# nagadomi/nunif

Hardware: NVIDIA H100
Metric: waifu2x_input_megapixels_per_sec (higher is better)
Workload: dtype f16

## Files before the change

### nunif_b200/csrc/gemm.cu

```cuda
#include "gemm.h"
#include "gemm_wgmma.cuh"
#include "tmap.h"
#include "../../include/nunif_b200.h"
#include <mutex>
#include <cstdlib>

namespace nb200 {

typedef CUresult (*EncodeTiledFn)(CUtensorMap*, CUtensorMapDataType, cuuint32_t, void*, const cuuint64_t*,
                                  const cuuint64_t*, const cuuint32_t*, const cuuint32_t*, CUtensorMapInterleave,
                                  CUtensorMapSwizzle, CUtensorMapL2promotion, CUtensorMapFloatOOBfill);

static EncodeTiledFn get_encode() {
    static EncodeTiledFn fn = nullptr;
    static std::once_flag once;
    std::call_once(once, [] {
        void* p = nullptr;
        cudaDriverEntryPointQueryResult q;
        if (cudaGetDriverEntryPoint("cuTensorMapEncodeTiled", &p, cudaEnableDefault, &q) == cudaSuccess &&
            q == cudaDriverEntryPointSuccess)
            fn = (EncodeTiledFn)p;
    });
    return fn;
}

int encode(CUtensorMap* m, const void* base, int rank, const cuuint64_t* dims, const cuuint64_t* strides_bytes,
                  const cuuint32_t* box, int swizzle_bytes) {
    EncodeTiledFn fn = get_encode();
    if (!fn) return fail("cuTensorMapEncodeTiled is not available (no CUDA driver?)");
    cuuint32_t estr[5] = {1, 1, 1, 1, 1};
    CUtensorMapSwizzle sw = swizzle_bytes == 128 ? CU_TENSOR_MAP_SWIZZLE_128B
                                                 : (swizzle_bytes == 64 ? CU_TENSOR_MAP_SWIZZLE_64B : CU_TENSOR_MAP_SWIZZLE_32B);
    CUresult r = fn(m, CU_TENSOR_MAP_DATA_TYPE_FLOAT16, (cuuint32_t)rank, const_cast<void*>(base), dims, strides_bytes, box,
                    estr, CU_TENSOR_MAP_INTERLEAVE_NONE, sw, CU_TENSOR_MAP_L2_PROMOTION_L2_256B,
                    CU_TENSOR_MAP_FLOAT_OOB_FILL_NONE);
    if (r != CUDA_SUCCESS) return fail("cuTensorMapEncodeTiled failed with CUresult " + std::to_string((int)r));
    return 0;
}

template <int BN, int BK, bool A2 = false>
static int launch_t(cudaStream_t st, const GemmMaps& maps, const GemmParams& p, int m_tiles, int n_tiles) {
    using Cfg = GemmCfg<BN, BK>;
    if (ensure_dyn_smem((const void*)gemm_conv_kernel<BN, BK, A2>, Cfg::SMEM_BYTES)) return 1;
    cudaLaunchConfig_t cfg = {};
    cfg.gridDim = dim3((unsigned)m_tiles * n_tiles); cfg.blockDim = dim3(GEMM_THREADS); cfg.dynamicSmemBytes = Cfg::SMEM_BYTES;
    cfg.stream = st;
    cudaLaunchAttribute at[1];
    at[0].id = cudaLaunchAttributeProgrammaticStreamSerialization;
    at[0].val.programmaticStreamSerializationAllowed = 1;
    cfg.attrs = at; cfg.numAttrs = 1;
    NB_CUDA(cudaLaunchKernelEx(&cfg, gemm_conv_kernel<BN, BK, A2>, maps, p));
    NB_LAUNCHED();
    return 0;
}

template <int BK>
static int launch_bn(int bn, cudaStream_t st, const GemmMaps& maps, const GemmParams& p, int m_tiles, int n_tiles) {
    if (p.k2) switch (bn) {
        case 64: return launch_t<64, BK, true>(st, maps, p, m_tiles, n_tiles);
        case 96: return launch_t<96, BK, true>(st, maps, p, m_tiles, n_tiles);
        default: return fail("second A operand: unsupported BLOCK_N");
    }
    switch (bn) {
        case 16: return launch_t<16, BK>(st, maps, p, m_tiles, n_tiles);
        case 32: return launch_t<32, BK>(st, maps, p, m_tiles, n_tiles);
        case 48: return launch_t<48, BK>(st, maps, p, m_tiles, n_tiles);
        case 64: return launch_t<64, BK>(st, maps, p, m_tiles, n_tiles);
        case 96: return launch_t<96, BK>(st, maps, p, m_tiles, n_tiles);
        case 128: return launch_t<128, BK>(st, maps, p, m_tiles, n_tiles);
    }
    return fail("unsupported BLOCK_N");
}

static int num_sms() { return device_sm_count(); }

std::atomic<int> g_tune_epoch{0};
int g_tune[16] = {0, 0, 0,  0, 0, 0,  0,
                   0, 0,  0,
                   0,
                   0, 0, 0, 0, 0};

static int encode_nhwc4(CUtensorMap* m, const __half* base, int C, int X, int Y, int B, long long sx, long long sy, long long sb,
                        int cw, int tw, int th) {
    cuuint64_t dims[4] = {(cuuint64_t)C, (cuuint64_t)X, (cuuint64_t)Y, (cuuint64_t)B};
    cuuint64_t strides[3] = {(cuuint64_t)sx * 2, (cuuint64_t)sy * 2, (cuuint64_t)sb * 2};
    cuuint32_t box[4] = {(cuuint32_t)cw, (cuuint32_t)tw, (cuuint32_t)th, 1};
    return encode(m, base, 4, dims, strides, box, cw * 2);
}

int conv_gemm(cudaStream_t st, const ConvGemm& g) {
    NB_CHECK(g.A && g.Wt && g.out, "null pointer");
    NB_CHECK(g.Ci % 8 == 0, "input channel stride must be a multiple of 8");
    NB_CHECK(g.N % 16 == 0, "N must be a multiple of 16 (pad the weights)");
    GemmParams p;
    memset(&p, 0, sizeof(p));
    int ktap;
    cuuint64_t dims[5], strides[4];
    cuuint32_t box[5];
    const cuuint64_t e = 2;
    const cuuint64_t rs = (g.a_row_stride ? (cuuint64_t)g.a_row_stride : (cuuint64_t)g.Wi * g.Ci) * e;
    const cuuint64_t is = (g.a_img_stride ? (cuuint64_t)g.a_img_stride * e : (cuuint64_t)g.Hi * rs);
    switch (g.kind) {
        case CG_LINEAR_FLAT: {
            const long long M = (long long)g.B * g.Hi * g.Wi;
            p.B = 1; p.Ho = 1; p.Wo = (int)M; p.TH = 1; p.TW = 128;
            p.taps = g.a_planes; ktap = g.Cin;
            NB_CHECK(g.a_planes >= 1 && g.a_planes <= 16, "bad plane count");
            for (int t = 0; t < p.taps; ++t) { p.tap_dy[t] = 0; p.tap_dx[t] = 0; p.tap_dyi[t] = (int8_t)t; }
            dims[0] = g.Cin; dims[1] = M; dims[2] = g.a_planes; dims[3] = 1; dims[4] = 1;
            strides[0] = g.Ci * e; strides[1] = (g.a_planes > 1 ? (cuuint64_t)g.a_plane_stride : (cuuint64_t)M * g.Ci) * e;
            strides[2] = (cuuint64_t)M * g.Ci * e * g.a_planes; strides[3] = strides[2];
            break;
        }
        case CG_LINEAR_2D:
        case CG_CONV3: {
            const int kk = g.kind == CG_CONV3 ? 3 : 1;
            const int pad = g.kind == CG_CONV3 ? g.pad : 0;
            NB_CHECK(pad == 0 || pad == 1, "conv3x3 padding must be 0 or 1");
            p.B = g.B; p.Ho = g.Hi - (kk - 1) + 2 * pad; p.Wo = g.Wi - (kk - 1) + 2 * pad; p.TH = 8; p.TW = 16;
            p.taps = kk * kk; ktap = g.Cin;
            for (int t = 0; t < p.taps; ++t) { p.tap_dy[t] = (int8_t)(t / kk - pad); p.tap_dx[t] = (int8_t)(t % kk - pad); p.tap_dyi[t] = 0; }
            dims[0] = g.Cin; dims[1] = g.Wi; dims[2] = 1; dims[3] = g.Hi; dims[4] = g.B;
            strides[0] = g.Ci * e; strides[1] = rs; strides[2] = rs;
            strides[3] = is;
            break;
        }
        case CG_TCONV3: {
            NB_CHECK(g.dil >= 1 && g.dil <= 127, "temporal dilation must be in [1, 127]");
            p.B = g.B; p.Ho = g.Hi; p.Wo = g.Wi; p.TH = 8; p.TW = 16;
            p.taps = 3; ktap = g.Cin;
            for (int t = 0; t < 3; ++t) { p.tap_dy[t] = (int8_t)((t - 1) * g.dil); p.tap_dx[t] = 0; p.tap_dyi[t] = 0; }
            dims[0] = g.Cin; dims[1] = g.Wi; dims[2] = 1; dims[3] = g.Hi; dims[4] = g.B;
            strides[0] = g.Ci * e; strides[1] = rs; strides[2] = rs;
// ... 56 lines not shown
            if (c >= bn || g.N % c) continue;
            const int w = (c % 64 == 0) ? 64 : 32;
            if (split && g.cout % w) continue;
            bn = c; cw = w;
        }
    }
    p.n_tiles = g.N / bn;
    box[0] = BK; box[1] = p.TW; box[2] = 1; box[3] = p.TH; box[4] = 1;
    GemmMaps maps;
    memset(&maps, 0, sizeof(maps));
    if (encode(&maps.a, g.A, 5, dims, strides, box, BK * 2)) return 1;
    const int K = p.taps * ktap + (a2 ? g.Cin2 : 0);
    cuuint64_t bdims[2] = {(cuuint64_t)K, (cuuint64_t)g.N};
    cuuint64_t bstr[1] = {(cuuint64_t)K * e};
    cuuint32_t bbox[2] = {(cuuint32_t)BK, (cuuint32_t)bn};
    if (encode(&maps.b, g.Wt, 2, bdims, bstr, bbox, BK * 2)) return 1;
    if (split) {
        for (int q = 0; q < g.N / g.cout; ++q)
            if (encode_nhwc4(&maps.o[q], g.out + (size_t)q * g.split_stride, g.cout, p.Wo, p.Ho, p.B, g.ldo, (long long)p.Wo * g.ldo,
                             (long long)p.Ho * p.Wo * g.ldo, cw, p.TW, p.TH)) return 1;
    } else if (!shuf) {
        if (encode_nhwc4(&maps.o[0], g.out, g.N, p.Wo, p.Ho, p.B, g.ldo, (long long)p.Wo * g.ldo, (long long)p.Ho * p.Wo * g.ldo,
                         cw, p.TW, p.TH)) return 1;
        if (g.res) {
            const int rW = g.kind == CG_LINEAR_FLAT ? p.Wo : g.res_W, rH = g.kind == CG_LINEAR_FLAT ? 1 : g.res_H;
            p.res_cx = g.kind == CG_LINEAR_FLAT ? 0 : g.res_cx;
            p.res_cy = g.kind == CG_LINEAR_FLAT ? 0 : g.res_cy;
            if (encode_nhwc4(&maps.r[0], g.res, g.N, rW, rH, p.B, g.ldr, (long long)rW * g.ldr, (long long)rH * rW * g.ldr, cw,
                             p.TW, p.TH)) return 1;
        }
    } else {
        const int OW = 2 * p.Wo, OH = 2 * p.Ho;
        for (int q = 0; q < 4; ++q) {
            const int dy = q >> 1, dx = q & 1;
            if (encode_nhwc4(&maps.o[q], g.out + ((size_t)dy * OW + dx) * g.ldo, g.cout, p.Wo, p.Ho, p.B, 2LL * g.ldo,
                             2LL * OW * g.ldo, (long long)OH * OW * g.ldo, cw, p.TW, p.TH)) return 1;
            if (g.res) {
                const int oy = dy + g.res_cy, ox = dx + g.res_cx;
                NB_CHECK(oy + 2 * (p.Ho - 1) < g.res_H && ox + 2 * (p.Wo - 1) < g.res_W, "residual tensor too small");
                if (encode_nhwc4(&maps.r[q], g.res + ((size_t)oy * g.res_W + ox) * g.ldr, g.cout, p.Wo, p.Ho, p.B, 2LL * g.ldr,
                                 2LL * g.res_W * g.ldr, (long long)g.res_H * g.res_W * g.ldr, cw, p.TW, p.TH)) return 1;
            }
        }
        p.res_cx = p.res_cy = 0;
        if (a2) {
            const cuuint64_t px = (cuuint64_t)g.ld2 * e;
            cuuint64_t d2[5] = {(cuuint64_t)g.Cin2, 2, (cuuint64_t)p.Wo, 2, (cuuint64_t)p.B * p.Ho};
            cuuint64_t s2[4] = {px, 2 * px, (cuuint64_t)OW * px, 2 * (cuuint64_t)OW * px};
            cuuint32_t b2[5] = {(cuuint32_t)BK, 1, (cuuint32_t)p.TW, 1, (cuuint32_t)p.TH};
            if (encode(&maps.a2, g.A2, 5, d2, s2, b2, BK * 2)) return 1;
        }
    }
    const int m_tiles = p.tiles_x * p.tiles_y * p.B;
    const double Mrows = (double)p.B * p.Ho * p.Wo;
    const double in_px = g.kind == CG_DOWN2 ? 4.0 * Mrows : ((g.kind == CG_CONV3 || g.kind == CG_TCONV3) ? (double)p.B * g.Hi * g.Wi : Mrows);
    ProfScope ps(st, PC_GEMM, 2.0 * Mrows * (double)g.N * (double)K,
                 in_px * (g.kind == CG_LINEAR_FLAT ? g.Cin * g.a_planes : g.Cin) * 2.0 + (g.res ? Mrows * g.N * 2.0 : 0.0) +
                     4.0 * Mrows * g.Cin2 * (a2 ? 2.0 : 0.0) + (double)g.N * K * 2.0,
                 Mrows * (double)g.N * 2.0);
    if (rec_on())
        rec_launch("gemm", {{"kind", g.kind}, {"pad", g.pad}, {"dil", g.dil}, {"B", g.B}, {"Hi", g.Hi}, {"Wi", g.Wi}, {"Ci", g.Ci},
                            {"Cin", g.Cin}, {"a_row_stride", g.a_row_stride}, {"a_img_stride", g.a_img_stride},
                            {"a_planes", g.a_planes}, {"a_plane_stride", g.a_plane_stride}, {"N", g.N}, {"act", g.act},
                            {"ldo", g.ldo}, {"out_mode", g.out_mode}, {"cout", g.cout}, {"split_stride", g.split_stride},
                            {"has_bias", g.bias ? 1 : 0}, {"has_res", g.res ? 1 : 0}, {"ldr", g.ldr}, {"res_H", g.res_H},
                            {"res_W", g.res_W}, {"res_cy", g.res_cy}, {"res_cx", g.res_cx}, {"res_before_act", g.res_before_act},
                            {"has_a2", a2 ? 1 : 0}, {"Cin2", g.Cin2}, {"ld2", g.ld2},
                            {"out_is_res", g.res && (const void*)g.out == (const void*)g.res},
                            {"out_is_a", (const void*)g.out == (const void*)g.A}, {"block_n", bn}, {"bk", BK},
                            {"grid", m_tiles * p.n_tiles}});
    return BK == 64 ? launch_bn<64>(bn, st, maps, p, m_tiles, p.n_tiles) : launch_bn<32>(bn, st, maps, p, m_tiles, p.n_tiles);
}

}

using namespace nb200;

extern "C" int nb200_conv_gemm_f16(const void* A, int B, int Hi, int Wi, int Ci, int Cin, int kind, const void* Wt, int N,
                                   const float* bias, int act, void* out, int ldo, int out_mode, int cout,
                                   const void* res, int ldr, int res_H, int res_W, int res_cy, int res_cx,
                                   int res_before_act, void* stream) {
    ConvGemm g;
    g.A = (const __half*)A; g.B = B; g.Hi = Hi; g.Wi = Wi; g.Ci = Ci; g.Cin = Cin;
    g.kind = kind == 4 ? CG_CONV3 : kind;
    g.pad = kind == 4 ? 1 : 0;
    g.Wt = (const __half*)Wt; g.N = N; g.bias = bias; g.act = act; g.out = (__half*)out; g.ldo = ldo;
    g.out_mode = out_mode; g.cout = cout; g.res = (const __half*)res; g.ldr = ldr; g.res_H = res_H; g.res_W = res_W;
    g.res_cy = res_cy; g.res_cx = res_cx; g.res_before_act = res_before_act;
    return conv_gemm((cudaStream_t)stream, g);
}

extern "C" int nb200_conv_gemm_pixshuf_a2_f16(const void* A, int B, int Hi, int Wi, int Ci, const void* Wt, int N, const float* bias,
                                              int act, void* out, int ldo, int cout, const void* A2, int Cin2, int ld2, void* stream) {
    ConvGemm g;
    g.A = (const __half*)A; g.B = B; g.Hi = Hi; g.Wi = Wi; g.Ci = Ci; g.Cin = Ci; g.kind = CG_LINEAR_2D;
    g.Wt = (const __half*)Wt; g.N = N; g.bias = bias; g.act = act; g.out = (__half*)out; g.ldo = ldo;
    g.out_mode = OUT_PIXSHUF2; g.cout = cout; g.A2 = (const __half*)A2; g.Cin2 = Cin2; g.ld2 = ld2;
    NB_CHECK(g.A2, "null pointer");
    return conv_gemm((cudaStream_t)stream, g);
}

extern "C" int nb200_conv_gemm_ex_f16(const nb200_gemm_desc* d, const void* A, const void* Wt, const float* bias, void* out,
                                      const void* res, const void* A2, void* stream) {
    NB_CHECK(d, "null descriptor");
    ConvGemm g;
    g.A = (const __half*)A; g.B = d->B; g.Hi = d->Hi; g.Wi = d->Wi; g.Ci = d->Ci; g.Cin = d->Cin;
    g.a_row_stride = d->a_row_stride; g.a_img_stride = d->a_img_stride; g.kind = d->kind; g.pad = d->pad; g.dil = d->dil;
    g.Wt = (const __half*)Wt; g.N = d->N; g.bias = bias; g.act = d->act; g.out = (__half*)out; g.ldo = d->ldo;
    g.out_mode = d->out_mode; g.cout = d->cout; g.split_stride = d->split_stride; g.a_planes = d->a_planes;
    g.a_plane_stride = d->a_plane_stride; g.res = (const __half*)res; g.ldr = d->ldr; g.res_H = d->res_H; g.res_W = d->res_W;
    g.res_cy = d->res_cy; g.res_cx = d->res_cx; g.res_before_act = d->res_before_act;
    g.A2 = (const __half*)A2; g.Cin2 = d->Cin2; g.ld2 = d->ld2;
    return conv_gemm((cudaStream_t)stream, g);
}

extern "C" int nb200_tune_set(int key, int value) {
    NB_CHECK(key >= 0 && key < 16, "bad key");
    g_tune[key] = value;
    g_tune_epoch.fetch_add(1);
    return 0;
}
```

### nunif_b200/csrc/gemm_wgmma.cuh

```cuda
#pragma once
#include "common.cuh"
#include "ptx.cuh"
#include <cuda.h>

namespace nb200 {

enum : int { ACT_NONE = 0, ACT_LRELU01 = 1, ACT_GELU = 2, ACT_RELU = 3 };
enum : int { OUT_NHWC = 0, OUT_PIXSHUF2 = 1, OUT_SPLIT = 2 };

struct GemmParams {
    int B, Ho, Wo, TH, TW, tiles_x, tiles_y;
    int N;
    int taps, cpt;
    int8_t tap_dx[16], tap_dy[16], tap_dyi[16];
    int n_tiles;
    const float* bias;
    int act;
    int out_mode, cout;
    int has_res, res_cy, res_cx;
    int res_before_act;
    int k2;
};

struct GemmMaps {
// ... 121 lines not shown
template <> __device__ __forceinline__ void wgmma_f16<128>(float (&d)[64], uint64_t a, uint64_t b, uint32_t acc) {
    asm volatile("{\n\t.reg .pred p;\n\tsetp.ne.b32 p, %66, 0;\n\t"
                 "wgmma.mma_async.sync.aligned.m64n128k16.f32.f16.f16 {%0, %1, %2, %3, %4, %5, %6, %7, %8, %9, %10, %11, %12, %13, %14, %15, %16, %17, %18, %19, %20, %21, %22, %23, %24, %25, %26, %27, %28, %29, %30, %31, %32, %33, %34, %35, %36, %37, %38, %39, %40, %41, %42, %43, %44, %45, %46, %47, %48, %49, %50, %51, %52, %53, %54, %55, %56, %57, %58, %59, %60, %61, %62, %63}, %64, %65, p, 1, 1, 0, 0;\n\t}"
                 : "+f"(d[0]), "+f"(d[1]), "+f"(d[2]), "+f"(d[3]), "+f"(d[4]), "+f"(d[5]), "+f"(d[6]), "+f"(d[7]), "+f"(d[8]), "+f"(d[9]), "+f"(d[10]), "+f"(d[11]), "+f"(d[12]), "+f"(d[13]), "+f"(d[14]), "+f"(d[15]), "+f"(d[16]), "+f"(d[17]), "+f"(d[18]), "+f"(d[19]), "+f"(d[20]), "+f"(d[21]), "+f"(d[22]), "+f"(d[23]), "+f"(d[24]), "+f"(d[25]), "+f"(d[26]), "+f"(d[27]), "+f"(d[28]), "+f"(d[29]), "+f"(d[30]), "+f"(d[31]), "+f"(d[32]), "+f"(d[33]), "+f"(d[34]), "+f"(d[35]), "+f"(d[36]), "+f"(d[37]), "+f"(d[38]), "+f"(d[39]), "+f"(d[40]), "+f"(d[41]), "+f"(d[42]), "+f"(d[43]), "+f"(d[44]), "+f"(d[45]), "+f"(d[46]), "+f"(d[47]), "+f"(d[48]), "+f"(d[49]), "+f"(d[50]), "+f"(d[51]), "+f"(d[52]), "+f"(d[53]), "+f"(d[54]), "+f"(d[55]), "+f"(d[56]), "+f"(d[57]), "+f"(d[58]), "+f"(d[59]), "+f"(d[60]), "+f"(d[61]), "+f"(d[62]), "+f"(d[63])
                 : "l"(a), "l"(b), "r"(acc));
}

__device__ __forceinline__ void wgmma_f16_rs96(float (&d)[48], const uint32_t (&a)[4], uint64_t b, uint32_t acc) {
    asm volatile("{\n\t.reg .pred p;\n\tsetp.ne.b32 p, %53, 0;\n\t"
                 "wgmma.mma_async.sync.aligned.m64n96k16.f32.f16.f16 {%0, %1, %2, %3, %4, %5, %6, %7, %8, %9, %10, %11, %12, %13, %14, %15, %16, %17, %18, %19, %20, %21, %22, %23, %24, %25, %26, %27, %28, %29, %30, %31, %32, %33, %34, %35, %36, %37, %38, %39, %40, %41, %42, %43, %44, %45, %46, %47}, {%48, %49, %50, %51}, %52, p, 1, 1, 0;\n\t}"
                 : "+f"(d[0]), "+f"(d[1]), "+f"(d[2]), "+f"(d[3]), "+f"(d[4]), "+f"(d[5]), "+f"(d[6]), "+f"(d[7]), "+f"(d[8]), "+f"(d[9]), "+f"(d[10]), "+f"(d[11]), "+f"(d[12]), "+f"(d[13]), "+f"(d[14]), "+f"(d[15]), "+f"(d[16]), "+f"(d[17]), "+f"(d[18]), "+f"(d[19]), "+f"(d[20]), "+f"(d[21]), "+f"(d[22]), "+f"(d[23]), "+f"(d[24]), "+f"(d[25]), "+f"(d[26]), "+f"(d[27]), "+f"(d[28]), "+f"(d[29]), "+f"(d[30]), "+f"(d[31]), "+f"(d[32]), "+f"(d[33]), "+f"(d[34]), "+f"(d[35]), "+f"(d[36]), "+f"(d[37]), "+f"(d[38]), "+f"(d[39]), "+f"(d[40]), "+f"(d[41]), "+f"(d[42]), "+f"(d[43]), "+f"(d[44]), "+f"(d[45]), "+f"(d[46]), "+f"(d[47])
                 : "r"(a[0]), "r"(a[1]), "r"(a[2]), "r"(a[3]), "l"(b), "r"(acc));
}

__device__ __forceinline__ float gelu_erf(float x) {
    const float a = fabsf(x);
    float q = fmaf(a, 4.88118734e-04f, -7.19881030e-03f);
    q = fmaf(q, a, 5.21468017e-02f);
    q = fmaf(q, a, 4.59595724e-01f);
    q = fmaf(q, a, 1.15100057e+00f);
    const float e = ex2(fmaf(-q, a, -1.0f));
    return fmaxf(x, 0.f) - a * e;
}

template <int K>
__device__ __forceinline__ void apply_act(float (&v)[K], int act) {
    switch (act) {
        case ACT_LRELU01:
#pragma unroll
            for (int j = 0; j < K; ++j) v[j] = v[j] > 0.f ? v[j] : 0.1f * v[j];
            break;
        case ACT_GELU:
#pragma unroll
            for (int j = 0; j < K; ++j) v[j] = gelu_erf(v[j]);
            break;
        case ACT_RELU:
#pragma unroll
            for (int j = 0; j < K; ++j) v[j] = fmaxf(v[j], 0.f);
            break;
        default: break;
    }
}

constexpr int GEMM_CONSUMER_THREADS = 256;
constexpr int GEMM_THREADS = GEMM_CONSUMER_THREADS + 32;

template <int BLOCK_N, int BK>
struct GemmCfg {
    static_assert(BLOCK_N % 16 == 0 && BLOCK_N <= 128, "BLOCK_N: 16..128 (the fp32 accumulators live in registers)");
    static constexpr int SWIZZLE = BK * 2;
    static constexpr int A_BYTES = 128 * BK * 2;
    static constexpr int B_BYTES = BLOCK_N * BK * 2;
    static constexpr int STAGE_BYTES = A_BYTES + ((B_BYTES + 1023) / 1024) * 1024;
    static constexpr int STAGES = (98304 / STAGE_BYTES) < 2 ? 2 : ((98304 / STAGE_BYTES) > 6 ? 6 : (98304 / STAGE_BYTES));
    static constexpr int CW = (BLOCK_N % 64 == 0) ? 64 : ((BLOCK_N % 32 == 0) ? 32 : 16);
    static constexpr int NCH = BLOCK_N / CW;
    static constexpr int CH_BYTES = 128 * CW * 2;
    static_assert(NCH * CH_BYTES <= STAGES * STAGE_BYTES, "epilogue staging must fit in the (drained) pipeline stages");
    static constexpr int SMEM_BYTES = STAGES * STAGE_BYTES + 1024  + 256 ;
};

template <int CW>
__device__ __forceinline__ uint32_t stage_off(int r, int j) {
    if (CW == 64) return (uint32_t)(r * 128 + ((j ^ (r & 7)) << 4));
    if (CW == 32) return (uint32_t)(r * 64 + ((j ^ ((r >> 1) & 3)) << 4));
    return (uint32_t)(r * 32 + ((j ^ ((r >> 2) & 1)) << 4));
}

template <int ROWS>
__device__ __forceinline__ uint32_t sw64_off(int r, int col) {
    return (uint32_t)((col >> 5) * (ROWS * 64)) + stage_off<32>(r, (col & 31) >> 3) + (uint32_t)((col & 7) * 2);
}

template <int BLOCK_N, int BK, bool A2 = false>
__global__ void __launch_bounds__(GEMM_THREADS, 2) gemm_conv_kernel(const __grid_constant__ GemmMaps maps,
                                                                    const __grid_constant__ GemmParams p) {
    using Cfg = GemmCfg<BLOCK_N, BK>;
    constexpr int STAGES = Cfg::STAGES;
    constexpr int CW = Cfg::CW;
    extern __shared__ uint8_t smem_dyn[];
    uint8_t* smem = reinterpret_cast<uint8_t*>((reinterpret_cast<uintptr_t>(smem_dyn) + 1023) & ~(uintptr_t)1023);
    uint64_t* full_bar = reinterpret_cast<uint64_t*>(smem + STAGES * Cfg::STAGE_BYTES);
    uint64_t* empty_bar = full_bar + STAGES;
    uint64_t* res_bar = empty_bar + STAGES;

    const int warp = threadIdx.x >> 5;
    const int n_tile = blockIdx.x % p.n_tiles;
    const int tile = blockIdx.x / p.n_tiles;
    const int tx_i = tile % p.tiles_x;
    const int ty_i = (tile / p.tiles_x) % p.tiles_y;
    const int b = tile / (p.tiles_x * p.tiles_y);
    const int x0 = tx_i * p.TW, y0 = ty_i * p.TH;
    const int n0 = n_tile * BLOCK_N;
    const int k_iters = p.taps * p.cpt + (A2 ? p.k2 : 0);

    if (threadIdx.x == GEMM_CONSUMER_THREADS) {
        tma_prefetch_desc(&maps.a);
        tma_prefetch_desc(&maps.b);
        tma_prefetch_desc(&maps.o[0]);
        for (int s = 0; s < STAGES; ++s) {
            mbar_init(&full_bar[s], 1);
            mbar_init(&empty_bar[s], 2);
        }
        mbar_init(res_bar, 1);
        fence_barrier_init();
    }
    __syncthreads();

    if (warp == GEMM_CONSUMER_THREADS / 32) {
        if (elect_one()) {
            asm volatile("griddepcontrol.wait;" ::: "memory");
            for (int it = 0; it < k_iters; ++it) {
                const int s = it % STAGES;
                const uint32_t ph = (it / STAGES) & 1;
                mbar_wait(&empty_bar[s], ph ^ 1);
                const int tap = it / p.cpt, ch = it - tap * p.cpt;
                uint8_t* sa = smem + s * Cfg::STAGE_BYTES;
                uint8_t* sb = sa + Cfg::A_BYTES;
                mbar_expect_tx(&full_bar[s], Cfg::A_BYTES + Cfg::B_BYTES);
                if (A2 && tap >= p.taps) {
                    const int q = n0 / p.cout;
                    tma_load_5d(&maps.a2, &full_bar[s], sa, (it - p.taps * p.cpt) * BK, q & 1, x0, q >> 1, b * p.Ho + y0);
                } else {
                    tma_load_5d(&maps.a, &full_bar[s], sa, ch * BK, x0 + p.tap_dx[tap], p.tap_dyi[tap], y0 + p.tap_dy[tap], b);
                }
                tma_load_2d(&maps.b, &full_bar[s], sb, it * BK, n0);
            }
        }
        return;
    }

    const int wg = threadIdx.x >> 7;
    const int t = threadIdx.x & 127;
    float acc[BLOCK_N / 2];
#pragma unroll
    for (int j = 0; j < BLOCK_N / 2; ++j) acc[j] = 0.f;
    for (int it = 0; it < k_iters; ++it) {
        const int s = it % STAGES;
        mbar_wait(&full_bar[s], (it / STAGES) & 1);
        const uint32_t sa = smem_u32(smem + s * Cfg::STAGE_BYTES) + wg * 64 * Cfg::SWIZZLE;
        const uint32_t sb = smem_u32(smem + s * Cfg::STAGE_BYTES) + Cfg::A_BYTES;
        wgmma_fence();
#pragma unroll
        for (int k = 0; k < BK / 16; ++k)
            wgmma_f16<BLOCK_N>(acc, make_kmajor_desc<Cfg::SWIZZLE>(sa + k * 32), make_kmajor_desc<Cfg::SWIZZLE>(sb + k * 32), 1u);
        wgmma_commit();
        wgmma_wait<1>();
        if (it > 0 && t == 0) mbar_arrive(&empty_bar[(it - 1) % STAGES]);
    }
    wgmma_wait<0>();
    wgmma_fence_operands(acc);
    if (threadIdx.x == 0) NB_PDL_TRIGGER();
    consumer_bar_sync();
    uint8_t* stg = smem;
    const bool leader = threadIdx.x == 0;
    if (p.has_res) {
        if (leader) {
            mbar_expect_tx(res_bar, Cfg::NCH * Cfg::CH_BYTES);
#pragma unroll 1
            for (int c = 0; c < Cfg::NCH; ++c) {
                const int n = n0 + c * CW;
                const int g = p.out_mode != OUT_NHWC ? n / p.cout : 0;
                const int co = p.out_mode != OUT_NHWC ? n - g * p.cout : n;
                tma_load_4d(&maps.r[g], res_bar, stg + c * Cfg::CH_BYTES, co, x0 + p.res_cx, y0 + p.res_cy, b);
            }
        }
        mbar_wait(res_bar, 0);
    }
    const int act = p.act;
    const bool has_res = p.has_res != 0, res_first = p.res_before_act != 0;
    const int row0 = wg * 64 + (t >> 5) * 16 + ((t & 31) >> 2);
    const int cq = 2 * (t & 3);
#pragma unroll
    for (int j = 0; j < BLOCK_N / 8; ++j) {
        const int col = 8 * j + cq;
        const int c = (8 * j) / CW;
        float2 bq = make_float2(0.f, 0.f);
        if (p.bias) bq = __ldg(reinterpret_cast<const float2*>(p.bias + n0 + col));
        float v[4] = {acc[4 * j] + bq.x, acc[4 * j + 1] + bq.y, acc[4 * j + 2] + bq.x, acc[4 * j + 3] + bq.y};
        __half2* s0 = reinterpret_cast<__half2*>(stg + c * Cfg::CH_BYTES + stage_off<CW>(row0, (8 * j % CW) / 8) + 2 * cq);
        __half2* s1 = reinterpret_cast<__half2*>(stg + c * Cfg::CH_BYTES + stage_off<CW>(row0 + 8, (8 * j % CW) / 8) + 2 * cq);
        if (has_res) {
            const float2 r0 = __half22float2(*s0), r1 = __half22float2(*s1);
            const float rv[4] = {r0.x, r0.y, r1.x, r1.y};
            if (res_first) {
#pragma unroll
                for (int q = 0; q < 4; ++q) v[q] += rv[q];
                apply_act(v, act);
            } else {
                apply_act(v, act);
#pragma unroll
                for (int q = 0; q < 4; ++q) v[q] += rv[q];
            }
        } else {
            apply_act(v, act);
        }
        *s0 = __floats2half2_rn(v[0], v[1]);
        *s1 = __floats2half2_rn(v[2], v[3]);
    }
    fence_async_smem();
    consumer_bar_sync();
    if (leader) {
#pragma unroll 1
        for (int c = 0; c < Cfg::NCH; ++c) {
            const int n = n0 + c * CW;
            const int g = p.out_mode != OUT_NHWC ? n / p.cout : 0;
            const int co = p.out_mode != OUT_NHWC ? n - g * p.cout : n;
            tma_store_4d(&maps.o[g], stg + c * Cfg::CH_BYTES, co, x0, y0, b);
        }
        tma_store_commit();
        tma_store_wait_read();
    }
}

}
```

Baseline: 79.55.

## Make wgmma conv GEMM persistent with dedicated epilogue staging buffer

Turns the conv GEMM kernel into a persistent kernel. The grid is capped at two CTAs per SM and each CTA loops over tiles, so the producer's TMA ring keeps prefetching the next tile while the consumers run the epilogue. A separate staging buffer for the epilogue lets output TMA stores overlap with the next tile's mainloop, and the PDL trigger moves to kernel start. The trade-off is fewer pipeline stages, since shared memory is sized for two CTAs per SM, plus extra cross-tile barrier phase tracking that could hurt small or low-tile-count layers.

```diff
diff --git a/nunif_b200/csrc/gemm.cu b/nunif_b200/csrc/gemm.cu
--- a/nunif_b200/csrc/gemm.cu
+++ b/nunif_b200/csrc/gemm.cu
@@ -2,6 +2,7 @@
 #include "gemm_wgmma.cuh"
 #include "tmap.h"
 #include "../../include/nunif_b200.h"
+#include <algorithm>
 #include <mutex>
 #include <cstdlib>
 
@@ -39,11 +40,11 @@
 }
 
 template <int BN, int BK, bool A2 = false>
-static int launch_t(cudaStream_t st, const GemmMaps& maps, const GemmParams& p, int m_tiles, int n_tiles) {
+static int launch_t(cudaStream_t st, const GemmMaps& maps, const GemmParams& p, int grid) {
     using Cfg = GemmCfg<BN, BK>;
     if (ensure_dyn_smem((const void*)gemm_conv_kernel<BN, BK, A2>, Cfg::SMEM_BYTES)) return 1;
     cudaLaunchConfig_t cfg = {};
-    cfg.gridDim = dim3((unsigned)m_tiles * n_tiles); cfg.blockDim = dim3(GEMM_THREADS); cfg.dynamicSmemBytes = Cfg::SMEM_BYTES;
+    cfg.gridDim = dim3((unsigned)grid); cfg.blockDim = dim3(GEMM_THREADS); cfg.dynamicSmemBytes = Cfg::SMEM_BYTES;
     cfg.stream = st;
     cudaLaunchAttribute at[1];
     at[0].id = cudaLaunchAttributeProgrammaticStreamSerialization;
@@ -55,19 +56,19 @@
 }
 
 template <int BK>
-static int launch_bn(int bn, cudaStream_t st, const GemmMaps& maps, const GemmParams& p, int m_tiles, int n_tiles) {
+static int launch_bn(int bn, cudaStream_t st, const GemmMaps& maps, const GemmParams& p, int grid) {
     if (p.k2) switch (bn) {
-        case 64: return launch_t<64, BK, true>(st, maps, p, m_tiles, n_tiles);
-        case 96: return launch_t<96, BK, true>(st, maps, p, m_tiles, n_tiles);
+        case 64: return launch_t<64, BK, true>(st, maps, p, grid);
+        case 96: return launch_t<96, BK, true>(st, maps, p, grid);
         default: return fail("second A operand: unsupported BLOCK_N");
     }
     switch (bn) {
-        case 16: return launch_t<16, BK>(st, maps, p, m_tiles, n_tiles);
-        case 32: return launch_t<32, BK>(st, maps, p, m_tiles, n_tiles);
-        case 48: return launch_t<48, BK>(st, maps, p, m_tiles, n_tiles);
-        case 64: return launch_t<64, BK>(st, maps, p, m_tiles, n_tiles);
-        case 96: return launch_t<96, BK>(st, maps, p, m_tiles, n_tiles);
-        case 128: return launch_t<128, BK>(st, maps, p, m_tiles, n_tiles);
+        case 16: return launch_t<16, BK>(st, maps, p, grid);
+        case 32: return launch_t<32, BK>(st, maps, p, grid);
+        case 48: return launch_t<48, BK>(st, maps, p, grid);
+        case 64: return launch_t<64, BK>(st, maps, p, grid);
+        case 96: return launch_t<96, BK>(st, maps, p, grid);
+        case 128: return launch_t<128, BK>(st, maps, p, grid);
     }
     return fail("unsupported BLOCK_N");
 }
@@ -78,7 +79,8 @@
 int g_tune[16] = {0, 0, 0,  0, 0, 0,  0,
                    0, 0,  0,
                    0,
-                   0, 0, 0, 0, 0};
+                   0,
+                   0, 0, 0, 0};
 
 static int encode_nhwc4(CUtensorMap* m, const __half* base, int C, int X, int Y, int B, long long sx, long long sy, long long sb,
                         int cw, int tw, int th) {
@@ -241,6 +243,8 @@
         }
     }
     const int m_tiles = p.tiles_x * p.tiles_y * p.B;
+    int grid = std::min(m_tiles * p.n_tiles, 2 * num_sms());
+    if (g_tune[12] > 0) grid = std::min(grid, g_tune[12]);
     const double Mrows = (double)p.B * p.Ho * p.Wo;
     const double in_px = g.kind == CG_DOWN2 ? 4.0 * Mrows : ((g.kind == CG_CONV3 || g.kind == CG_TCONV3) ? (double)p.B * g.Hi * g.Wi : Mrows);
     ProfScope ps(st, PC_GEMM, 2.0 * Mrows * (double)g.N * (double)K,
@@ -257,8 +261,8 @@
                             {"has_a2", a2 ? 1 : 0}, {"Cin2", g.Cin2}, {"ld2", g.ld2},
                             {"out_is_res", g.res && (const void*)g.out == (const void*)g.res},
                             {"out_is_a", (const void*)g.out == (const void*)g.A}, {"block_n", bn}, {"bk", BK},
-                            {"grid", m_tiles * p.n_tiles}});
-    return BK == 64 ? launch_bn<64>(bn, st, maps, p, m_tiles, p.n_tiles) : launch_bn<32>(bn, st, maps, p, m_tiles, p.n_tiles);
+                            {"grid", grid}});
+    return BK == 64 ? launch_bn<64>(bn, st, maps, p, grid) : launch_bn<32>(bn, st, maps, p, grid);
 }
 
 }
diff --git a/nunif_b200/csrc/gemm_wgmma.cuh b/nunif_b200/csrc/gemm_wgmma.cuh
--- a/nunif_b200/csrc/gemm_wgmma.cuh
+++ b/nunif_b200/csrc/gemm_wgmma.cuh
@@ -197,12 +197,16 @@
     static constexpr int A_BYTES = 128 * BK * 2;
     static constexpr int B_BYTES = BLOCK_N * BK * 2;
     static constexpr int STAGE_BYTES = A_BYTES + ((B_BYTES + 1023) / 1024) * 1024;
-    static constexpr int STAGES = (98304 / STAGE_BYTES) < 2 ? 2 : ((98304 / STAGE_BYTES) > 6 ? 6 : (98304 / STAGE_BYTES));
     static constexpr int CW = (BLOCK_N % 64 == 0) ? 64 : ((BLOCK_N % 32 == 0) ? 32 : 16);
     static constexpr int NCH = BLOCK_N / CW;
     static constexpr int CH_BYTES = 128 * CW * 2;
-    static_assert(NCH * CH_BYTES <= STAGES * STAGE_BYTES, "epilogue staging must fit in the (drained) pipeline stages");
-    static constexpr int SMEM_BYTES = STAGES * STAGE_BYTES + 1024  + 256 ;
+    static constexpr int STG_BYTES = NCH * CH_BYTES;
+    static constexpr int SMEM_PER_CTA = (228 * 1024 - 2 * 1024) / 2;
+    static constexpr int RING_FIT = (SMEM_PER_CTA - 1024  - 256  - STG_BYTES) / STAGE_BYTES;
+    static constexpr int STAGES = RING_FIT > 6 ? 6 : RING_FIT;
+    static_assert(STAGES >= 2, "the ring needs two stages beside the staging tile");
+    static constexpr int SMEM_BYTES = STAGES * STAGE_BYTES + STG_BYTES + 1024  + 256 ;
+    static_assert(SMEM_BYTES <= SMEM_PER_CTA, "two CTAs per SM");
 };
 
 template <int CW>
@@ -215,6 +219,16 @@
 template <int ROWS>
 __device__ __forceinline__ uint32_t sw64_off(int r, int col) {
     return (uint32_t)((col >> 5) * (ROWS * 64)) + stage_off<32>(r, (col & 31) >> 3) + (uint32_t)((col & 7) * 2);
+}
+
+struct GemmTile { int x0, y0, b, n0; };
+template <int BLOCK_N>
+__device__ __forceinline__ GemmTile gemm_tile(const GemmParams& p, int idx) {
+    const int n_tile = idx % p.n_tiles;
+    const int tile = idx / p.n_tiles;
+    const int tx_i = tile % p.tiles_x;
+    const int ty_i = (tile / p.tiles_x) % p.tiles_y;
+    return {tx_i * p.TW, ty_i * p.TH, tile / (p.tiles_x * p.tiles_y), n_tile * BLOCK_N};
 }
 
 template <int BLOCK_N, int BK, bool A2 = false>
@@ -225,18 +239,13 @@
     constexpr int CW = Cfg::CW;
     extern __shared__ uint8_t smem_dyn[];
     uint8_t* smem = reinterpret_cast<uint8_t*>((reinterpret_cast<uintptr_t>(smem_dyn) + 1023) & ~(uintptr_t)1023);
-    uint64_t* full_bar = reinterpret_cast<uint64_t*>(smem + STAGES * Cfg::STAGE_BYTES);
+    uint8_t* stg = smem + STAGES * Cfg::STAGE_BYTES;
+    uint64_t* full_bar = reinterpret_cast<uint64_t*>(stg + Cfg::STG_BYTES);
     uint64_t* empty_bar = full_bar + STAGES;
     uint64_t* res_bar = empty_bar + STAGES;
 
     const int warp = threadIdx.x >> 5;
-    const int n_tile = blockIdx.x % p.n_tiles;
-    const int tile = blockIdx.x / p.n_tiles;
-    const int tx_i = tile % p.tiles_x;
-    const int ty_i = (tile / p.tiles_x) % p.tiles_y;
-    const int b = tile / (p.tiles_x * p.tiles_y);
-    const int x0 = tx_i * p.TW, y0 = ty_i * p.TH;
-    const int n0 = n_tile * BLOCK_N;
+    const int n_tiles_all = p.tiles_x * p.tiles_y * p.B * p.n_tiles;
     const int k_iters = p.taps * p.cpt + (A2 ? p.k2 : 0);
 
     if (threadIdx.x == GEMM_CONSUMER_THREADS) {
@@ -251,25 +260,34 @@
         fence_barrier_init();
     }
     __syncthreads();
+    if (threadIdx.x == 0) NB_PDL_TRIGGER();
 
     if (warp == GEMM_CONSUMER_THREADS / 32) {
         if (elect_one()) {
             asm volatile("griddepcontrol.wait;" ::: "memory");
-            for (int it = 0; it < k_iters; ++it) {
-                const int s = it % STAGES;
-                const uint32_t ph = (it / STAGES) & 1;
-                mbar_wait(&empty_bar[s], ph ^ 1);
-                const int tap = it / p.cpt, ch = it - tap * p.cpt;
-                uint8_t* sa = smem + s * Cfg::STAGE_BYTES;
-                uint8_t* sb = sa + Cfg::A_BYTES;
-                mbar_expect_tx(&full_bar[s], Cfg::A_BYTES + Cfg::B_BYTES);
-                if (A2 && tap >= p.taps) {
-                    const int q = n0 / p.cout;
-                    tma_load_5d(&maps.a2, &full_bar[s], sa, (it - p.taps * p.cpt) * BK, q & 1, x0, q >> 1, b * p.Ho + y0);
-                } else {
-                    tma_load_5d(&maps.a, &full_bar[s], sa, ch * BK, x0 + p.tap_dx[tap], p.tap_dyi[tap], y0 + p.tap_dy[tap], b);
+            int s = 0;
+            uint32_t ph = 0;
+#pragma unroll 1
+            for (int idx = blockIdx.x; idx < n_tiles_all; idx += gridDim.x) {
+                const GemmTile tl = gemm_tile<BLOCK_N>(p, idx);
+#pragma unroll 1
+                for (int it = 0; it < k_iters; ++it) {
+                    mbar_wait(&empty_bar[s], ph ^ 1);
+                    const int tap = it / p.cpt, ch = it - tap * p.cpt;
+                    uint8_t* sa = smem + s * Cfg::STAGE_BYTES;
+                    uint8_t* sb = sa + Cfg::A_BYTES;
+                    mbar_expect_tx(&full_bar[s], Cfg::A_BYTES + Cfg::B_BYTES);
+                    if (A2 && tap >= p.taps) {
+                        const int q = tl.n0 / p.cout;
+                        tma_load_5d(&maps.a2, &full_bar[s], sa, (it - p.taps * p.cpt) * BK, q & 1, tl.x0, q >> 1,
+                                    tl.b * p.Ho + tl.y0);
+                    } else {
+                        tma_load_5d(&maps.a, &full_bar[s], sa, ch * BK, tl.x0 + p.tap_dx[tap], p.tap_dyi[tap],
+                                    tl.y0 + p.tap_dy[tap], tl.b);
+                    }
+                    tma_load_2d(&maps.b, &full_bar[s], sb, it * BK, tl.n0);
+                    if (++s == STAGES) { s = 0; ph ^= 1; }
                 }
-                tma_load_2d(&maps.b, &full_bar[s], sb, it * BK, n0);
             }
         }
         return;
@@ -277,85 +295,95 @@
 
     const int wg = threadIdx.x >> 7;
     const int t = threadIdx.x & 127;
-    float acc[BLOCK_N / 2];
-#pragma unroll
-    for (int j = 0; j < BLOCK_N / 2; ++j) acc[j] = 0.f;
-    for (int it = 0; it < k_iters; ++it) {
-        const int s = it % STAGES;
-        mbar_wait(&full_bar[s], (it / STAGES) & 1);
-        const uint32_t sa = smem_u32(smem + s * Cfg::STAGE_BYTES) + wg * 64 * Cfg::SWIZZLE;
-        const uint32_t sb = smem_u32(smem + s * Cfg::STAGE_BYTES) + Cfg::A_BYTES;
-        wgmma_fence();
-#pragma unroll
-        for (int k = 0; k < BK / 16; ++k)
-            wgmma_f16<BLOCK_N>(acc, make_kmajor_desc<Cfg::SWIZZLE>(sa + k * 32), make_kmajor_desc<Cfg::SWIZZLE>(sb + k * 32), 1u);
-        wgmma_commit();
-        wgmma_wait<1>();
-        if (it > 0 && t == 0) mbar_arrive(&empty_bar[(it - 1) % STAGES]);
-    }
-    wgmma_wait<0>();
-    wgmma_fence_operands(acc);
-    if (threadIdx.x == 0) NB_PDL_TRIGGER();
-    consumer_bar_sync();
-    uint8_t* stg = smem;
     const bool leader = threadIdx.x == 0;
-    if (p.has_res) {
-        if (leader) {
-            mbar_expect_tx(res_bar, Cfg::NCH * Cfg::CH_BYTES);
-#pragma unroll 1
-            for (int c = 0; c < Cfg::NCH; ++c) {
-                const int n = n0 + c * CW;
-                const int g = p.out_mode != OUT_NHWC ? n / p.cout : 0;
-                const int co = p.out_mode != OUT_NHWC ? n - g * p.cout : n;
-                tma_load_4d(&maps.r[g], res_bar, stg + c * Cfg::CH_BYTES, co, x0 + p.res_cx, y0 + p.res_cy, b);
-            }
-        }
-        mbar_wait(res_bar, 0);
-    }
     const int act = p.act;
     const bool has_res = p.has_res != 0, res_first = p.res_before_act != 0;
     const int row0 = wg * 64 + (t >> 5) * 16 + ((t & 31) >> 2);
     const int cq = 2 * (t & 3);
-#pragma unroll
-    for (int j = 0; j < BLOCK_N / 8; ++j) {
-        const int col = 8 * j + cq;
-        const int c = (8 * j) / CW;
-        float2 bq = make_float2(0.f, 0.f);
-        if (p.bias) bq = __ldg(reinterpret_cast<const float2*>(p.bias + n0 + col));
-        float v[4] = {acc[4 * j] + bq.x, acc[4 * j + 1] + bq.y, acc[4 * j + 2] + bq.x, acc[4 * j + 3] + bq.y};
-        __half2* s0 = reinterpret_cast<__half2*>(stg + c * Cfg::CH_BYTES + stage_off<CW>(row0, (8 * j % CW) / 8) + 2 * cq);
-        __half2* s1 = reinterpret_cast<__half2*>(stg + c * Cfg::CH_BYTES + stage_off<CW>(row0 + 8, (8 * j % CW) / 8) + 2 * cq);
+    int s = 0;
+    uint32_t ph = 0, res_ph = 0;
+#pragma unroll 1
+    for (int idx = blockIdx.x; idx < n_tiles_all; idx += gridDim.x) {
+        const GemmTile tl = gemm_tile<BLOCK_N>(p, idx);
+        float acc[BLOCK_N / 2];
+#pragma unroll
+        for (int j = 0; j < BLOCK_N / 2; ++j) acc[j] = 0.f;
+        int prev = 0;
+        for (int it = 0; it < k_iters; ++it) {
+            mbar_wait(&full_bar[s], ph);
+            const uint32_t sa = smem_u32(smem + s * Cfg::STAGE_BYTES) + wg * 64 * Cfg::SWIZZLE;
+            const uint32_t sb = smem_u32(smem + s * Cfg::STAGE_BYTES) + Cfg::A_BYTES;
+            wgmma_fence();
+#pragma unroll
+            for (int k = 0; k < BK / 16; ++k)
+                wgmma_f16<BLOCK_N>(acc, make_kmajor_desc<Cfg::SWIZZLE>(sa + k * 32), make_kmajor_desc<Cfg::SWIZZLE>(sb + k * 32), 1u);
+            wgmma_commit();
+            wgmma_wait<1>();
+            if (it > 0 && t == 0) mbar_arrive(&empty_bar[prev]);
+            prev = s;
+            if (++s == STAGES) { s = 0; ph ^= 1; }
+        }
+        wgmma_wait<0>();
+        wgmma_fence_operands(acc);
+        if (t == 0) mbar_arrive(&empty_bar[prev]);
+
+        if (leader) tma_store_wait_read();
+        consumer_bar_sync();
         if (has_res) {
-            const float2 r0 = __half22float2(*s0), r1 = __half22float2(*s1);
-            const float rv[4] = {r0.x, r0.y, r1.x, r1.y};
-            if (res_first) {
-#pragma unroll
-                for (int q = 0; q < 4; ++q) v[q] += rv[q];
-                apply_act(v, act);
+            if (leader) {
+                mbar_expect_tx(res_bar, Cfg::STG_BYTES);
+#pragma unroll 1
+                for (int c = 0; c < Cfg::NCH; ++c) {
+                    const int n = tl.n0 + c * CW;
+                    const int g = p.out_mode != OUT_NHWC ? n / p.cout : 0;
+                    const int co = p.out_mode != OUT_NHWC ? n - g * p.cout : n;
+                    tma_load_4d(&maps.r[g], res_bar, stg + c * Cfg::CH_BYTES, co, tl.x0 + p.res_cx, tl.y0 + p.res_cy, tl.b);
+                }
+            }
+            mbar_wait(res_bar, res_ph);
+            res_ph ^= 1;
+        }
+#pragma unroll
+        for (int j = 0; j < BLOCK_N / 8; ++j) {
+            const int col = 8 * j + cq;
+            const int c = (8 * j) / CW;
+            float2 bq = make_float2(0.f, 0.f);
+            if (p.bias) bq = __ldg(reinterpret_cast<const float2*>(p.bias + tl.n0 + col));
+            float v[4] = {acc[4 * j] + bq.x, acc[4 * j + 1] + bq.y, acc[4 * j + 2] + bq.x, acc[4 * j + 3] + bq.y};
+            __half2* s0 = reinterpret_cast<__half2*>(stg + c * Cfg::CH_BYTES + stage_off<CW>(row0, (8 * j % CW) / 8) + 2 * cq);
+            __half2* s1 = reinterpret_cast<__half2*>(stg + c * Cfg::CH_BYTES + stage_off<CW>(row0 + 8, (8 * j % CW) / 8) + 2 * cq);
+            if (has_res) {
+                const float2 r0 = __half22float2(*s0), r1 = __half22float2(*s1);
+                const float rv[4] = {r0.x, r0.y, r1.x, r1.y};
+                if (res_first) {
+#pragma unroll
+                    for (int q = 0; q < 4; ++q) v[q] += rv[q];
+                    apply_act(v, act);
+                } else {
+                    apply_act(v, act);
+#pragma unroll
+                    for (int q = 0; q < 4; ++q) v[q] += rv[q];
+                }
             } else {
                 apply_act(v, act);
-#pragma unroll
-                for (int q = 0; q < 4; ++q) v[q] += rv[q];
             }
-        } else {
-            apply_act(v, act);
-        }
-        *s0 = __floats2half2_rn(v[0], v[1]);
-        *s1 = __floats2half2_rn(v[2], v[3]);
+            *s0 = __floats2half2_rn(v[0], v[1]);
+            *s1 = __floats2half2_rn(v[2], v[3]);
+        }
+        fence_async_smem();
+        consumer_bar_sync();
+        if (leader) {
+#pragma unroll 1
+            for (int c = 0; c < Cfg::NCH; ++c) {
+                const int n = tl.n0 + c * CW;
+                const int g = p.out_mode != OUT_NHWC ? n / p.cout : 0;
+                const int co = p.out_mode != OUT_NHWC ? n - g * p.cout : n;
+                tma_store_4d(&maps.o[g], stg + c * Cfg::CH_BYTES, co, tl.x0, tl.y0, tl.b);
+            }
+            tma_store_commit();
+        }
     }
-    fence_async_smem();
-    consumer_bar_sync();
-    if (leader) {
-#pragma unroll 1
-        for (int c = 0; c < Cfg::NCH; ++c) {
-            const int n = n0 + c * CW;
-            const int g = p.out_mode != OUT_NHWC ? n / p.cout : 0;
-            const int co = p.out_mode != OUT_NHWC ? n - g * p.cout : n;
-            tma_store_4d(&maps.o[g], stg + c * Cfg::CH_BYTES, co, x0, y0, b);
-        }
-        tma_store_commit();
-        tma_store_wait_read();
-    }
-}
-
-}
+    if (leader) tma_store_wait_read();
+}
+
+}
diff --git a/profiles/ab_gemm.py b/profiles/ab_gemm.py
--- /dev/null
+++ b/profiles/ab_gemm.py
@@ -0,0 +1,185 @@
+#!/usr/bin/env python
+import argparse
+import ctypes
+import json
+import os
+import statistics
+import subprocess
+import sys
+
+ROOT = os.path.dirname(os.path.dirname(os.path.abspath(__file__)))
+sys.path.insert(0, ROOT)
+
+REPS = 7
+WINDOW_MS = 60.0
+TENSOR_RATE = 650e12
+HBM_RATE = 3.35e12
+CONV3, LINEAR_2D, DOWN2 = 2, 1, 3
+LRELU, PIXSHUF2 = 1, 1
+
+SHAPES = [
+    ("swin4x conv2 3x3 64->96 240^2", dict(kind=CONV3, B=16, Hi=242, Wi=242, Ci=64, Cin=64, N=96, act=LRELU, ldo=96), None, None),
+    ("swin4x down1 2x2s2 96->192", dict(kind=DOWN2, B=16, Hi=240, Wi=240, Ci=96, Cin=96, N=192, ldo=192), None, None),
+    ("swin4x down2 2x2s2 192->192", dict(kind=DOWN2, B=16, Hi=120, Wi=120, Ci=192, Cin=192, N=192, ldo=192), None, None),
+    ("swin4x up2 + x4 (pixel shuffle)", dict(kind=LINEAR_2D, B=16, Hi=60, Wi=60, Ci=192, Cin=192, N=768, ldo=192,
+                                             out_mode=PIXSHUF2, cout=192, ldr=192, res_H=120, res_W=120), (120, 120), None),
+    ("swin4x up1 + proj2 (A2, pixel shuffle)", dict(kind=LINEAR_2D, B=16, Hi=120, Wi=120, Ci=192, Cin=192, N=768, ldo=192,
+                                                    out_mode=PIXSHUF2, cout=192, Cin2=96, ld2=96), None, (240, 240)),
+    ("upcunet 3x3 64->64 122^2", dict(kind=CONV3, B=16, Hi=124, Wi=124, Ci=64, Cin=64, N=64, act=LRELU, ldo=64), None, None),
+    ("upcunet 3x3 128->128 60^2", dict(kind=CONV3, B=16, Hi=62, Wi=62, Ci=128, Cin=128, N=128, act=LRELU, ldo=128), None, None),
+]
+
+
+def load(path):
+    from nunif_b200 import _lib
+    lib = ctypes.CDLL(os.path.abspath(path))
+    for name in ("nb200_last_error", "nb200_check_device", "nb200_conv_gemm_ex_f16"):
+        res, args = _lib.SIGNATURES[name]
+        getattr(lib, name).restype, getattr(lib, name).argtypes = res, args
+    return lib
+
+
+def check(lib, rc):
+    if rc != 0:
+        raise RuntimeError(lib.nb200_last_error().decode("utf-8", "replace"))
+
+
+def out_shape(f):
+    B, Hi, Wi = f["B"], f["Hi"], f["Wi"]
+    Ho, Wo = {CONV3: (Hi - 2, Wi - 2), DOWN2: (Hi // 2, Wi // 2), LINEAR_2D: (Hi, Wi)}[f["kind"]]
+    if f.get("out_mode") == PIXSHUF2:
+        return B, 2 * Ho, 2 * Wo, f["cout"]
+    return B, Ho, Wo, f["N"]
+
+
+def work(f):
+    B, Hi, Wi = f["B"], f["Hi"], f["Wi"]
+    taps_k = {CONV3: 9 * f["Cin"], DOWN2: 4 * f["Cin"], LINEAR_2D: f["Cin"]}[f["kind"]]
+    K = taps_k + f.get("Cin2", 0)
+    ob, oh, ow, oc = out_shape(f)
+    M = ob * oh * ow * oc // f["N"]
+    nbytes = 2 * (B * Hi * Wi * f["Cin"] + f["N"] * K + ob * oh * ow * oc)
+    if f.get("ldr"):
+        nbytes += 2 * ob * oh * ow * oc
+    if f.get("Cin2"):
+        nbytes += 2 * ob * oh * ow * f["Cin2"]
+    return 2.0 * M * f["N"] * K, float(nbytes)
+
+
+def inputs(i, f, res_hw, a2_hw, dev):
+    import torch
+    g = torch.Generator(device="cpu").manual_seed(1000 + i)
+    K = {CONV3: 9 * f["Cin"], DOWN2: 4 * f["Cin"], LINEAR_2D: f["Cin"]}[f["kind"]] + f.get("Cin2", 0)
+    t = {"A": torch.randn(f["B"], f["Hi"], f["Wi"], f["Ci"], generator=g).half().to(dev),
+         "Wt": (torch.randn(f["N"], K, generator=g) / K ** 0.5).half().to(dev),
+         "bias": (0.1 * torch.randn(f["N"], generator=g)).to(dev),
+         "out": torch.empty(out_shape(f), dtype=torch.float16, device=dev)}
+    t["res"] = torch.randn(f["B"], *res_hw, f["ldr"], generator=g).half().to(dev) if res_hw else None
+    t["A2"] = torch.randn(f["B"], *a2_hw, f["ld2"], generator=g).half().to(dev) if a2_hw else None
+    return t
+
+
+def call(lib, desc, t):
+    import torch
+    p = lambda v: ctypes.c_void_p(v.data_ptr() if v is not None else 0)
+    check(lib, lib.nb200_conv_gemm_ex_f16(ctypes.byref(desc), p(t["A"]), p(t["Wt"]), p(t["bias"]),
+                                          p(t["out"]), p(t["res"]), p(t["A2"]),
+                                          ctypes.c_void_p(torch.cuda.current_stream().cuda_stream)))
+
+
+def window_ms(lib, desc, t, n):
+    import torch
+    e0, e1 = torch.cuda.Event(enable_timing=True), torch.cuda.Event(enable_timing=True)
+    e0.record()
+    for _ in range(n):
+        call(lib, desc, t)
+    e1.record()
+    e1.synchronize()
+    return e0.elapsed_time(e1) / n
+
+
+def device_info(index):
+    q = subprocess.run(["nvidia-smi", "-i", str(index), "--query-gpu=name,power.limit,clocks.max.sm", "--format=csv,noheader"],
+                       capture_output=True, text=True)
+    return q.stdout.strip()
+
+
+def main():
+    ap = argparse.ArgumentParser(description=__doc__, formatter_class=argparse.RawDescriptionHelpFormatter)
+    ap.add_argument("--base", required=True, help="the build to compare against (libnunif_b200.so)")
+    ap.add_argument("--new", default=os.path.join(ROOT, "nunif_b200", "libnunif_b200.so"), help="default: this tree's build")
+    ap.add_argument("--out", default=None, help="also write the JSON result here")
+    args = ap.parse_args()
+    for p in (args.base, args.new):
+        if not os.path.isfile(p):
+            ap.error(f"no such library: {p}")
+    import torch
+    from bench import ClockSampler
+    from nunif_b200 import _lib
+    if not torch.cuda.is_available():
+        raise SystemExit("ab_gemm.py needs a CUDA device")
+    dev = torch.device("cuda:0")
+    torch.zeros(1, device=dev)
+    paths = {"base": args.base, "new": args.new}
+    libs = {k: load(v) for k, v in paths.items()}
+    for lib in libs.values():
+        check(lib, lib.nb200_check_device(0))
+    info = {"device": torch.cuda.get_device_name(dev), "nvidia_smi": device_info(0), "paths": paths}
+    print(f"# {info['device']} | name, power limit, max SM clock: {info['nvidia_smi']}")
+    print("| launch | M x N x K | GFLOP | MB | floor ms | base ms [min, max] | new ms [min, max] | new TFLOP/s | new GB/s | "
+          "new/base | outputs |")
+    print("|---|---|---|---|---|---|---|---|---|---|---|")
+
+    rows = []
+    with torch.inference_mode(), ClockSampler(0) as clocks:
+        for i, (name, fields, res_hw, a2_hw) in enumerate(SHAPES):
+            desc = _lib.GemmDesc(a_planes=1, **fields)
+            t = inputs(i, fields, res_hw, a2_hw, dev)
+            outs = {}
+            for k, lib in libs.items():
+                t["out"].fill_(float("nan"))
+                call(lib, desc, t)
+                torch.cuda.synchronize()
+                outs[k] = t["out"].clone()
+            equal = torch.equal(outs["base"].view(torch.int16), outs["new"].view(torch.int16))
+            del outs
+            for k, lib in libs.items():
+                for _ in range(3):
+                    call(lib, desc, t)
+            est = max(window_ms(libs["base"], desc, t, 3), window_ms(libs["new"], desc, t, 3))
+            n = max(5, int(WINDOW_MS / max(est, 1e-3)))
+            ms = {k: [] for k in libs}
+            for r in range(REPS):
+                for k in (("base", "new") if r % 2 == 0 else ("new", "base")):
+                    ms[k].append(window_ms(libs[k], desc, t, n))
+            flop, nbytes = work(fields)
+            floor = max(flop / TENSOR_RATE, nbytes / HBM_RATE) * 1e3
+            ob, oh, ow, oc = out_shape(fields)
+            M = ob * oh * ow * oc // fields["N"]
+            K = int(flop / (2.0 * M * fields["N"]))
+            row = {"name": name, "M": M, "N": fields["N"], "K": K, "gflop": flop / 1e9, "mbytes": nbytes / 1e6, "floor_ms": floor,
+                   "calls_per_window": n, "equal": equal}
+            for k in libs:
+                med = statistics.median(ms[k])
+                row[k] = {"median_ms": med, "min_ms": min(ms[k]), "max_ms": max(ms[k]), "tflops": flop / med / 1e9,
+                          "gbps": nbytes / med / 1e6}
+            row["new_over_base"] = row["new"]["median_ms"] / row["base"]["median_ms"]
+            rows.append(row)
+            b, nw = row["base"], row["new"]
+            print(f"| {name} | {M:,} x {fields['N']} x {K} | {flop / 1e9:.1f} | {nbytes / 1e6:.0f} | {floor:.3f} | "
+                  f"{b['median_ms']:.4f} [{b['min_ms']:.4f}, {b['max_ms']:.4f}] | "
+                  f"{nw['median_ms']:.4f} [{nw['min_ms']:.4f}, {nw['max_ms']:.4f}] | {nw['tflops']:.0f} | {nw['gbps']:.0f} | "
+                  f"{row['new_over_base']:.3f} | {'identical' if equal else 'DIFFER'} |", flush=True)
+            del t
+    result = {"info": info, "clocks": clocks.summary(), "shapes": rows, "all_equal": all(r["equal"] for r in rows)}
+    print(f"# SM clock during the timed region: {result['clocks']}")
+    print(json.dumps(result))
+    if args.out:
+        os.makedirs(os.path.dirname(os.path.abspath(args.out)), exist_ok=True)
+        with open(args.out, "w") as fh:
+            json.dump(result, fh, indent=1)
+    return 0 if result["all_equal"] else 1
+
+
+if __name__ == "__main__":
+    sys.exit(main())
```

After: 80.40, median of 6. 1.1% higher.
